# pbs-plus/pbs-plus

Hardware: AMD Instinct MI355X
Metric: GiB/s ingested through CDC+SHA-256 (higher is better)
Workload: dtype u32

## Files before the change

### go/pbsgpu/fallback.go

```go

package pbsgpu

import (
	"errors"
	"io"
	"unsafe"
)

var ErrNotBuilt = errors.New("pbsgpu: built without cgo/gpuchunk; GPU engine unavailable")

var (
	ErrBusy       = errors.New("pbsgpu: all in-flight tickets used")
	ErrHostFaster = errors.New("pbsgpu: too few files in flight for the GPU to beat host SHA-256; hash on the host")
)

const CommIDBytes = 128

type (
	Config struct {
		AvgSize, MinSize, MaxSize, WindowSize int
		BreakTestMask, BreakTestMinimum       uint32
	}
	ChunkInfo struct {
		End     uint64
// ... 22 lines not shown
		Encoded EncodeStats
	}
	ReuseChunk struct {
		Size, Padding, EndOffset uint64
		Digest                   [32]byte
	}
	FileHash    struct{ Index, Size, XXH3 uint64 }
	RingOptions struct {
		ArenaBytes, PageBytes                                                            uint64
		MaxStreams, ShaCUs, RoundPages                                                   uint32
		ExpressCUs                                                                       uint32
		MinRoundPages, MaxInflight, LongBytes, LongLoBytes, LongSpill, PollEvery, Flags uint32
		BacklogMiB, LoneDeferMs, IdleTimeoutS, AutoparkMs                                float64
		LanesCUs                                                                         uint32
		ShortBytes                                                                       uint64
		HoldPages                                                                        bool
	}
	EngineOptions struct {
		Inflight, ShaForm, ShaSlackPct, ShaDensePct                      uint32
		ResolveParMin                                                    uint64
		ShaManyFilesPerCore                                              uint32
		StreamShaCUs, StreamExpressCUs, StreamRingSlots, StreamCtxPool   uint32
		StreamRingGiB                                                    float64
		StreamPageBytes                                                  uint64
	}
	RingStats struct {
		PageBytes, BytesEnqueued, Chunks uint64
		PagesTotal, PagesFree, Rounds    uint32
		ServiceMsLast                    float64
	}
// ... 204 lines not shown
```

### go/pbsgpu/pbsgpu.go

```go

package pbsgpu

import "C"

import (
	"errors"
	"fmt"
	"io"
	"runtime"
	"unsafe"
)

type Config struct {
	AvgSize, MinSize, MaxSize, WindowSize int
	BreakTestMask, BreakTestMinimum       uint32
	c                                     C.pbsgpu_config
}

func NewConfig(avgSize int) (Config, error) {
	var cfg Config
	if st := C.pbsgpu_config_init(C.uint64_t(avgSize), nil, &cfg.c); st != C.PBSGPU_OK {
		return Config{}, fmt.Errorf("buzhash: invalid average chunk size %d: %s", avgSize, strerror(st))
	}
	cfg.AvgSize, cfg.MinSize, cfg.MaxSize = int(cfg.c.avg), int(cfg.c.min), int(cfg.c.max)
// ... 541 lines not shown


type Ring struct {
	h   *C.pbsgpu_ring
	eng *Engine
}

type RingOptions struct {
	ArenaBytes, PageBytes         uint64
	MaxStreams, ShaCUs, RoundPages uint32
	ExpressCUs uint32
	MinRoundPages, MaxInflight, LongBytes, LongLoBytes, LongSpill, PollEvery, Flags uint32
	BacklogMiB, LoneDeferMs, IdleTimeoutS, AutoparkMs                                float64
	LanesCUs   uint32
	ShortBytes uint64
	HoldPages bool
}

const RingOff = ^uint32(0)

func (e *Engine) NewRing(o RingOptions) (*Ring, error) {
	defer runtime.KeepAlive(e)
	co := C.pbsgpu_ring_options{arena_bytes: C.uint64_t(o.ArenaBytes), page_bytes: C.uint64_t(o.PageBytes),
		max_streams: C.uint32_t(o.MaxStreams), sha_cus: C.uint32_t(o.ShaCUs), round_pages: C.uint32_t(o.RoundPages),
		express_cus: C.uint32_t(o.ExpressCUs), min_round_pages: C.uint32_t(o.MinRoundPages),
		max_inflight: C.uint32_t(o.MaxInflight), long_bytes: C.uint32_t(o.LongBytes), long_lo_bytes: C.uint32_t(o.LongLoBytes),
		long_spill: C.uint32_t(o.LongSpill), poll_every: C.uint32_t(o.PollEvery), flags: C.uint32_t(o.Flags),
		backlog_mib: C.double(o.BacklogMiB), lone_defer_ms: C.double(o.LoneDeferMs), idle_timeout_s: C.double(o.IdleTimeoutS),
		autopark_ms: C.double(o.AutoparkMs), lanes_cus: C.uint32_t(o.LanesCUs), short_bytes: C.uint64_t(o.ShortBytes)}
	if o.HoldPages {
		co.flags |= C.PBSGPU_RING_F_HOLD_PAGES
	}
	r := &Ring{eng: e}
	if err := check(C.pbsgpu_ring_create(e.h, &co, &r.h), "ring_create"); err != nil {
		return nil, err
	}
	runtime.SetFinalizer(r, func(r *Ring) { r.Close() })
	return r, nil
}

func (r *Ring) Open() (uint32, error) {
	defer runtime.KeepAlive(r)
	var s C.uint32_t
	st := C.pbsgpu_ring_open(r.h, &s)
// ... 871 lines not shown
```

### include/pbsgpu.h

```cpp
#ifndef PBSGPU_H
#define PBSGPU_H

#include <stddef.h>
#include <stdint.h>

#ifdef __cplusplus
extern "C" {
#endif

#define PBSGPU_ABI_VERSION 5

#define PBSGPU_OK 0
#define PBSGPU_E_INVALID (-1)
#define PBSGPU_E_NO_DEVICE (-2)
#define PBSGPU_E_HIP (-3)
#define PBSGPU_E_NOMEM (-4)
#define PBSGPU_E_CAPACITY (-5)
#define PBSGPU_E_BUSY (-6)
#define PBSGPU_E_TICKET (-7)
#define PBSGPU_E_STATE (-9)

const char *pbsgpu_strerror(int status);
int pbsgpu_abi_version(void);
int pbsgpu_last_hip_error(void);
// ... 128 lines not shown
    uint32_t round_pages;
    uint32_t express_cus;
    uint32_t min_round_pages;
    uint32_t max_inflight;
    uint32_t long_bytes;
    uint32_t long_lo_bytes;
    uint32_t long_spill;
    uint32_t poll_every;
    uint32_t flags;
    uint32_t lanes_cus;
    double backlog_mib;
    double lone_defer_ms;
    double idle_timeout_s;
    double autopark_ms;
    uint64_t short_bytes;
    uint64_t reserved[3];
} pbsgpu_ring_options;
#define PBSGPU_RING_OFF 0xffffffffu
#define PBSGPU_RING_F_NO_OVERLAP 1u
#define PBSGPU_RING_F_NO_STAGE 2u
#define PBSGPU_RING_F_NO_CUT_PRIO 4u
#define PBSGPU_RING_F_NO_SPLIT_AUTO 8u
#define PBSGPU_RING_F_DEFER_SERVICE 16u
#define PBSGPU_RING_F_FILL_SERIAL 32u
#define PBSGPU_RING_F_DENSE_SERVICE 64u
#define PBSGPU_RING_F_DENSE_LANES 128u
#define PBSGPU_RING_F_TIER_TAG 256u
#define PBSGPU_RING_F_HOLD_PAGES 512u
typedef struct pbsgpu_ring_stats {
    uint64_t page_bytes, bytes_enqueued, chunks, candidates, pages_enqueued, pages_recycled, service_bytes_last;
    uint32_t pages_total, pages_free, sha_cus, rounds, rounds_done, rounds_in_flight, streams_opened, service_launches;
// ... 276 lines not shown
```

### pbs_plus_amd/_lib.py

```python
from __future__ import annotations

import ctypes as C
import os
import subprocess

import numpy as np

_HERE = os.path.dirname(os.path.abspath(__file__))
LIB_PATH = os.environ.get("PBSGPU_LIB_PATH") or os.path.join(_HERE, "lib", "libpbsgpu.so")
CSRC = os.path.join(_HERE, "csrc")

OK = 0
E_INVALID, E_NO_DEVICE, E_HIP, E_NOMEM, E_CAPACITY, E_BUSY, E_TICKET, _E_RETIRED_8, E_STATE = range(-1, -10, -1)


class PbsGpuError(RuntimeError):
    def __init__(self, status: int, what: str = ""):
        self.status = status
        msg = lib().pbsgpu_strerror(status).decode() if _lib is not None else str(status)
        hip = lib().pbsgpu_last_hip_error() if _lib is not None else 0
        extra = ""
        if _lib is not None and ("comm" in what or "allgather" in what):
            txt = lib().pbsgpu_comm_last_error()
            if txt:
# ... 53 lines not shown
RING_OFF = 0xFFFFFFFF
RING_F_NO_OVERLAP, RING_F_NO_STAGE, RING_F_NO_CUT_PRIO, RING_F_NO_SPLIT_AUTO, RING_F_DEFER_SERVICE, RING_F_FILL_SERIAL = 1, 2, 4, 8, 16, 32
RING_F_DENSE_SERVICE = 64
RING_F_DENSE_LANES = 128
RING_F_TIER_TAG = 256
RING_F_HOLD_PAGES = 512
RING_ANY_STREAM = 0xFFFFFFFF


class RingOptions(C.Structure):
    _fields_ = [("arena_bytes", C.c_uint64), ("page_bytes", C.c_uint64), ("max_streams", C.c_uint32),
                ("sha_cus", C.c_uint32), ("round_pages", C.c_uint32), ("express_cus", C.c_uint32),
                ("min_round_pages", C.c_uint32), ("max_inflight", C.c_uint32), ("long_bytes", C.c_uint32),
                ("long_lo_bytes", C.c_uint32), ("long_spill", C.c_uint32), ("poll_every", C.c_uint32), ("flags", C.c_uint32),
                ("lanes_cus", C.c_uint32), ("backlog_mib", C.c_double), ("lone_defer_ms", C.c_double),
                ("idle_timeout_s", C.c_double), ("autopark_ms", C.c_double), ("short_bytes", C.c_uint64), ("reserved", C.c_uint64 * 3)]


class EngineOptions(C.Structure):
    _fields_ = [("inflight", C.c_uint32), ("sha_form", C.c_uint32), ("sha_slack_pct", C.c_uint32), ("sha_dense_pct", C.c_uint32),
                ("resolve_par_min", C.c_uint64), ("sha_many_files_per_core", C.c_uint32), ("stream_sha_cus", C.c_uint32),
                ("stream_express_cus", C.c_uint32), ("stream_ring_slots", C.c_uint32), ("stream_ctx_pool", C.c_uint32),
                ("reserved0", C.c_uint32), ("stream_ring_gib", C.c_double), ("stream_page_bytes", C.c_uint64),
                ("reserved", C.c_uint64 * 4)]


class RingStats(C.Structure):
    _fields_ = [(k, C.c_uint64) for k in ("page_bytes", "bytes_enqueued", "chunks", "candidates", "pages_enqueued",
                                          "pages_recycled", "service_bytes_last")] + \
               [(k, C.c_uint32) for k in ("pages_total", "pages_free", "sha_cus", "rounds", "rounds_done",
                                          "rounds_in_flight", "streams_opened", "service_launches")] + \
# ... 222 lines not shown
```

### pbs_plus_amd/csrc/kernels.h

```cpp
#pragma once

#include <hip/hip_runtime.h>
#include <stdint.h>

#include "../../include/pbsgpu.h"

namespace pbsk {

constexpr int kWindow = 64;

struct ScanParams {
    const uint8_t *data_al;
    uint32_t lead;
    uint64_t nbytes;
    uint64_t ntiles;
    uint32_t tile_bytes;
    const uint32_t *table_rot;
    uint32_t thr;
    uint32_t cap;
    uint32_t *tile_cnt;
    uint32_t *tile_slots;
    unsigned long long *tile_queue;
    uint32_t tiles_per_wave;
    uint32_t shared_chip;
// ... 238 lines not shown
    const uint32_t *table_rot;
    const RingPage *pages;
    uint32_t npages;
    const RingSeg *segs_in;
    uint32_t nseg;
    uint32_t seq;
    uint32_t cell_base, cell_cap, cell_mask;
    uint32_t scan_blocks;
    RingRoundStatus *status;
    RingStreamState *streams;
    RingSource q;
    uint4 *desc_w;
    uint4 *ldesc_w;
    uint4 *sdesc_w;
    unsigned long long *tile_queue;
    uint32_t *scalars;
    uint32_t *tile_cnt, *tile_off, *tile_slots, *scan_tmp;
    uint64_t *dense;
    uint64_t dense_cap;
    pbsgpu_segment *segs;
    uint32_t *seg_cnt, *seg_off;
    pbsgpu_record *recs;
    uint64_t rec_cap;
    uint64_t *seg_newc;
    uint32_t *seg_open;
    uint64_t *seg_ecand_in;
    uint64_t *seg_ecand;
    const uint64_t *sugg;
    const uint32_t *sugg_idx;
    uint64_t sugg_feed;
    uint32_t sugg_abs;
    uint32_t pad0;
    const uint32_t *seg_rec_base;
};
struct RingStage {
    const uint8_t *src;
    uint8_t *dst;
    uint32_t off[4], len[4];
    const RingPage *pages_host;
};
hipError_t launch_ring_round(const RingRound &r, int num_cus, hipStream_t st, hipStream_t fill_st = nullptr,
                             hipEvent_t fill_ev = nullptr, hipStream_t scan_st = nullptr, hipEvent_t scan_ev = nullptr,
                             const RingStage *stage = nullptr);
hipError_t launch_ring_service(const RingSource &q, unsigned workgroups, hipStream_t st, bool dense = false);
hipError_t launch_ring_service_xp(const RingSource &q, unsigned workgroups, hipStream_t st);
hipError_t launch_ring_service_lanes(const RingSource &q, unsigned workgroups, hipStream_t st, bool dense);
hipError_t launch_ring_stop(RingCtl *ctl, hipStream_t st);
// ... 13 lines not shown
```

### pbs_plus_amd/csrc/ring.cpp

```cpp
#include <chrono>
#include <cstdio>
#include <cstdlib>
#include <thread>

#include "ring_internal.h"

using namespace pbse;

namespace {

double now_ms() {
    return std::chrono::duration<double, std::milli>(std::chrono::steady_clock::now().time_since_epoch()).count();
}

uint32_t pow2_at_least(uint64_t v) {
    uint32_t p = 1;
    while (p < v && p < (1u << 31)) p <<= 1;
    return p;
}

volatile uint32_t *hb_words(const pbsgpu_ring *r) { return r->heartbeat.as<volatile uint32_t>(); }

void ring_service_ended(pbsgpu_ring *r) {
    if (r->svc == SvcState::Stopped) return;
// ... 184 lines not shown
        if (inflight > 0 && !any_final && ready < r->min_round_pages) return PBSGPU_OK;
        if (inflight >= r->max_inflight) return PBSGPU_OK;
    }
    int in = -1;
    for (uint32_t i = 0; i < kRingInputs; ++i)
        if (!r->input_busy[i]) { in = (int)i; break; }
    if (in < 0) return PBSGPU_OK;
    {
        const uint64_t oldest = r->rounds.empty() ? r->cell_cursor : r->rounds.front().cell_base;
        if (r->cell_cursor + r->rec_cap - oldest > r->ncells) return PBSGPU_OK;
    }
    pbsk::RingPage *pg = r->in_pages((uint32_t)in);
    pbsk::RingSeg *sg = r->in_segs((uint32_t)in);
    uint32_t *recbase = r->in_recbase((uint32_t)in);
    uint32_t *suggidx = r->in_suggidx((uint32_t)in);
    uint32_t np = 0, ns = 0;
    uint64_t cells_needed = 0, new_bytes = 0;
    RoundInfo ri;
    std::vector<hipEvent_t> deps;
    std::vector<uint64_t> sugg;
    const uint32_t minsz = std::min(e->effmin, e->cfg.min);
    const uint64_t feed = e->sugg_feed.load(std::memory_order_relaxed);
    const uint64_t look = feed > 1 ? (uint64_t)e->cfg.max : 0;
    uint32_t streams_waiting = 0;
    for (auto &s : r->slots) streams_waiting += (s.open && !s.ready.empty()) ? 1u : 0u;
    const uint32_t round_cap = (r->svc == SvcState::Stopped || streams_waiting < 2)
                                   ? r->round_pages
                                   : std::max(std::min(r->round_pages, r->min_round_pages), r->round_pages / 2);
    for (uint32_t si = 0; si < r->slots.size() && np < round_cap; ++si) {
        StreamSlot &s = r->slots[si];
        if (!s.open || (s.ready.empty() && !s.zero_final)) continue;
// ... 3 lines not shown
        g.reset = s.fresh ? 1u : 0u;
        g.origin = s.origin;
        const uint64_t end_old = s.bytes_enqueued;
        uint64_t end = end_old;
        uint32_t take = 0;
        while (!s.ready.empty() && take < kPagesPerStreamRound && np < round_cap) {
            const PageReq &q = s.ready.front();
            pbsk::RingPage p{};
            p.phys = q.phys;
            p.phys_off = (uint64_t)q.phys * r->stride + 128u;
            p.logical = ((uint64_t)si << pbsk::kRingOffBits) | (q.k * r->page_bytes);
            p.valid = q.valid;
            p.slot = si;
            p.seg = ns;
            p.do_fill = q.do_fill ? 1u : 0u;
            p.fill_seed = q.seed;
            p.fill_off = q.fill_off;
            p.fill_kind = q.kind;
            p.fill_tab = q.tab;
            p.fill_ntab = q.ntab;
            p.prev_phys = (q.k > 0 && s.last_phys >= 0) ? (uint32_t)s.last_phys : 0xffffffffu;
            s.last_phys = (int64_t)q.phys;
            pg[np++] = p;
            if (q.dep) deps.push_back(q.dep);
            end += q.valid;
            new_bytes += q.valid;
            if (q.final) g.final = 1;
            s.ready.pop_front();
            ++take;
        }
// ... 75 lines not shown
    rr.nseg = ns;
    rr.seq = ri.seq;
    rr.cell_base = (uint32_t)(ri.cell_base & (r->ncells - 1));
    rr.cell_cap = ri.cell_cap;
    rr.cell_mask = r->ncells - 1;
    rr.scan_blocks = (uint32_t)std::max(1, e->num_cus - (int)r->svc_cus);
    rr.status = hs;
    rr.streams = r->streams.as<pbsk::RingStreamState>();
    rr.q = r->source();
    rr.desc_w = r->desc.as<uint4>();
    rr.ldesc_w = r->ldesc.as<uint4>();
    rr.sdesc_w = r->lanes_cus ? r->sdesc.as<uint4>() : nullptr;
    const uint32_t set = r->ps ? r->scan_set : 0u;
    rr.scalars = r->scalars.as<uint32_t>();
    rr.tile_queue = r->tileq.as<unsigned long long>() + set * 8u;
    rr.tile_cnt = set ? r->tile_cnt2.as<uint32_t>() : r->tile_cnt.as<uint32_t>();
    rr.tile_off = r->tile_off.as<uint32_t>();
    rr.tile_slots = set ? r->tile_slots2.as<uint32_t>() : r->tile_slots.as<uint32_t>();
    rr.scan_tmp = r->scan_tmp.as<uint32_t>();
    rr.dense = r->dense.as<uint64_t>();
    rr.dense_cap = r->dense_cap;
    rr.segs = r->segs.as<pbsgpu_segment>();
    rr.seg_cnt = r->seg_cnt.as<uint32_t>();
    rr.seg_off = r->seg_off.as<uint32_t>();
    rr.recs = r->recs.as<pbsgpu_record>();
    rr.rec_cap = r->rec_cap;
    rr.seg_newc = r->seg_newc.as<uint64_t>();
    rr.seg_open = r->seg_open.as<uint32_t>();
    rr.seg_ecand_in = r->seg_ecand_in.as<uint64_t>();
    rr.seg_ecand = r->seg_ecand.as<uint64_t>();
// ... 5 lines not shown
    std::atomic_thread_fence(std::memory_order_release);
    bool defer = r->defer_service;
    if (!defer && r->svc == SvcState::Stopped && r->lone_defer_ms > 0 && !any_final &&
        np >= std::max<uint32_t>(1, r->round_pages / 2)) {
        const uint64_t lanes_worth = (uint64_t)r->sha_cus * (r->dense_service ? 256u : 128u) * (uint64_t)e->cfg.avg;
        const double t = now_ms();
        if (r->defer_t0 == 0) r->defer_t0 = t;
        defer = t - r->defer_t0 < r->lone_defer_ms && r->deferred_bytes + new_bytes < lanes_worth;
    }
    if (!defer) {
        const int st = ring_start_service(r);
        if (st != PBSGPU_OK) return fail(st);
        rr.q = r->source();
    }
    if (r->svc == SvcState::Stopped) r->deferred_bytes += new_bytes;
    if (r->svc == SvcState::Stopped) rr.scan_blocks = (uint32_t)std::max(1, e->num_cus);
    else if (r->ps && rr.scan_blocks > 8) rr.scan_blocks -= 1;
    hipStream_t scan_st = r->ps ? r->ps : r->cs;
    for (hipEvent_t ev : deps)
        if (hipStreamWaitEvent(scan_st, ev, 0) != hipSuccess) return fail(PBSGPU_E_HIP);
    for (hipEvent_t ev : deps) ring_event_put(r, ev);
    deps.clear();
    if (r->ps && r->ctl_used[set])
        if (hipStreamWaitEvent(r->ps, r->ev_ctl[set], 0) != hipSuccess) return fail(PBSGPU_E_HIP);
    {
        const bool fill_serial = r->fill_serial;
        pbsk::RingStage stg{};
        if (r->stage_inputs) {
            const uint8_t *hb = r->in((uint32_t)in);
            uint8_t *db = r->in_dev((uint32_t)in);
            stg.src = hb;
            stg.dst = db;
            stg.off[0] = (uint32_t)r->in_pages_off;   stg.len[0] = np * (uint32_t)sizeof(pbsk::RingPage);
            stg.off[1] = (uint32_t)r->in_segs_off;    stg.len[1] = ns * (uint32_t)sizeof(pbsk::RingSeg);
            stg.off[2] = (uint32_t)r->in_recbase_off; stg.len[2] = (ns + 1u) * 4u;
            stg.off[3] = (uint32_t)r->in_suggidx_off; stg.len[3] = rr.sugg_idx ? (ns + 1u) * 4u : 0u;
            stg.pages_host = pg;
            auto mirror = [&](const void *hp) { return db + (reinterpret_cast<const uint8_t *>(hp) - hb); };
            rr.pages = reinterpret_cast<const pbsk::RingPage *>(mirror(pg));
            rr.segs_in = reinterpret_cast<const pbsk::RingSeg *>(mirror(sg));
            rr.seg_rec_base = reinterpret_cast<const uint32_t *>(mirror(recbase));
// ... 41 lines not shown
    enum Kind { U32, U32_ZERO_OFF, U64, F64, F64_ZERO_NEG, FLAG_IF_ZERO, FLAG_IF_SET };
    struct Entry {
        const char *name;
        Kind kind;
        void *field;
        uint32_t flag;
    };
    const Entry table[] = {
        {"PBSGPU_RING_SHA_CUS", U32, &o.sha_cus, 0},
        {"PBSGPU_RING_XP_CUS", U32_ZERO_OFF, &o.express_cus, 0},
        {"PBSGPU_RING_LANES_CUS", U32, &o.lanes_cus, 0},
        {"PBSGPU_RING_SHORT_BYTES", U64, &o.short_bytes, 0},
        {"PBSGPU_RING_ROUND_PAGES", U32, &o.round_pages, 0},
        {"PBSGPU_RING_MIN_ROUND_PAGES", U32, &o.min_round_pages, 0},
        {"PBSGPU_RING_MAX_INFLIGHT", U32, &o.max_inflight, 0},
        {"PBSGPU_RING_LONG_BYTES", U32_ZERO_OFF, &o.long_bytes, 0},
        {"PBSGPU_RING_LONG_LO_BYTES", U32_ZERO_OFF, &o.long_lo_bytes, 0},
        {"PBSGPU_RING_LONG_SPILL", U32, &o.long_spill, 0},
        {"PBSGPU_RING_POLL_EVERY", U32, &o.poll_every, 0},
        {"PBSGPU_RING_BACKLOG_MIB", F64_ZERO_NEG, &o.backlog_mib, 0},
        {"PBSGPU_RING_LONE_DEFER_MS", F64_ZERO_NEG, &o.lone_defer_ms, 0},
        {"PBSGPU_RING_IDLE_TIMEOUT_S", F64, &o.idle_timeout_s, 0},
        {"PBSGPU_RING_AUTOPARK_MS", F64, &o.autopark_ms, 0},
        {"PBSGPU_RING_OVERLAP", FLAG_IF_ZERO, &o.flags, PBSGPU_RING_F_NO_OVERLAP},
        {"PBSGPU_RING_STAGE_INPUTS", FLAG_IF_ZERO, &o.flags, PBSGPU_RING_F_NO_STAGE},
        {"PBSGPU_RING_CUT_PRIO", FLAG_IF_ZERO, &o.flags, PBSGPU_RING_F_NO_CUT_PRIO},
        {"PBSGPU_RING_SPLIT_AUTO", FLAG_IF_ZERO, &o.flags, PBSGPU_RING_F_NO_SPLIT_AUTO},
        {"PBSGPU_RING_DEFER_SERVICE", FLAG_IF_SET, &o.flags, PBSGPU_RING_F_DEFER_SERVICE},
        {"PBSGPU_RING_FILL_SERIAL", FLAG_IF_SET, &o.flags, PBSGPU_RING_F_FILL_SERIAL},
        {"PBSGPU_RING_DENSE_SERVICE", FLAG_IF_SET, &o.flags, PBSGPU_RING_F_DENSE_SERVICE},
// ... 204 lines not shown
                                               : std::max(1u, r->round_pages / 4);
        r->backlog_limit = o.backlog_mib < 0 ? 0 : o.backlog_mib > 0 ? (uint64_t)(o.backlog_mib * 1048576.0)   : (uint64_t)(r->sha_cus + r->lanes_cus) << 27;
        r->backlog_auto = o.backlog_mib == 0;
        if (o.max_inflight) r->max_inflight = std::min<uint32_t>(std::max(1u, o.max_inflight), kRingInputs);
        r->autopark_ms = std::max(0.0, o.autopark_ms);
        r->defer_service = (o.flags & PBSGPU_RING_F_DEFER_SERVICE) != 0;
        r->fill_serial = (o.flags & PBSGPU_RING_F_FILL_SERIAL) != 0;
        r->dense_service = (o.flags & PBSGPU_RING_F_DENSE_SERVICE) != 0;
        r->dense_lanes = (o.flags & PBSGPU_RING_F_DENSE_LANES) != 0;
        r->tier_tag = (o.flags & PBSGPU_RING_F_TIER_TAG) != 0;
        r->lone_defer_ms = o.lone_defer_ms < 0 ? 0.0 : o.lone_defer_ms > 0 ? o.lone_defer_ms : 25.0;
        r->idle_timeout_s = o.idle_timeout_s;
        r->opt_long_lo = o.long_lo_bytes;
        r->opt_long_spill = o.long_spill;
        r->opt_poll_every = o.poll_every;
        const double lambda = 3.0 * r->tile_bytes / ((double)e->cfg.mask + 1.0);
        uint32_t capv = 8;
        while (capv < 4.0 * lambda + 16.0) capv <<= 1;
        r->cap = std::min<uint32_t>(std::max<uint32_t>(capv * 2, r->tile_bytes / 128), r->tile_bytes);
        const uint64_t ntiles = (uint64_t)r->round_pages * r->tpp;
        if (ntiles * r->cap >= (1ull << 32)) return PBSGPU_E_INVALID;
        const uint32_t minsz = std::min(e->effmin, e->cfg.min);
        r->dense_cap = ntiles * r->cap;
        r->rec_cap = ((uint64_t)r->round_pages * r->page_bytes + (uint64_t)r->max_streams * e->cfg.max) / minsz +
                     4ull * r->max_streams + 64;
        const uint64_t resident_chunks = (uint64_t)r->npages * r->page_bytes / minsz + 2ull * r->npages + r->rec_cap;
        r->qslots = pow2_at_least(2 * resident_chunks + 4096);
        r->ncells = pow2_at_least(4 * resident_chunks + 4 * r->rec_cap);
        r->nfree = pow2_at_least(4ull * r->npages + 64);

// ... 3 lines not shown
        CHK(r->streams.ensure((size_t)r->max_streams * sizeof(pbsk::RingStreamState)));
        CHK(r->pending.ensure((size_t)r->npages * 4 + 64));
        CHK(r->desc.ensure((size_t)r->qslots * 32));
        r->long_bytes = r->xp_cus ? (long_bytes_hint ? long_bytes_hint : (uint32_t)((uint64_t)e->cfg.max * 13 / 16)) : 0;
        r->long_lo_auto = long_bytes_hint == 0;
        if (o.long_bytes) r->long_bytes = o.long_bytes == PBSGPU_RING_OFF ? 0u : o.long_bytes;
        if (r->xp_cus && r->long_bytes == 0) r->xp_cus = 0;
        r->lslots = pow2_at_least(2 * ((uint64_t)r->npages * r->page_bytes / std::max<uint32_t>(r->long_bytes, minsz) + r->rec_cap) + 1024);
        CHK(r->ldesc.ensure((size_t)r->lslots * 32));
        r->sslots = r->lanes_cus ? r->qslots : 2;
        CHK(r->sdesc.ensure((size_t)r->sslots * 32));
        CHK(r->scalars.ensure(pbsk::kRsCount * 4 + 64));
        CHK(r->tile_cnt.ensure((size_t)ntiles * 4 + 16));
        CHK(r->tile_off.ensure((size_t)ntiles * 4 + 16));
        CHK(r->tile_slots.ensure((size_t)ntiles * r->cap * 4 + 16));
        CHK(r->tileq.ensure(128));
        const bool overlap = !(o.flags & PBSGPU_RING_F_NO_OVERLAP);
        if (overlap) {
            CHK(r->tile_cnt2.ensure((size_t)ntiles * 4 + 16));
            CHK(r->tile_slots2.ensure((size_t)ntiles * r->cap * 4 + 16));
        }
        CHK(r->dense.ensure((size_t)r->dense_cap * 8 + 16));
        CHK(r->scan_tmp.ensure(pbsk::scan_tmp_words(std::max<uint64_t>(ntiles, r->max_streams)) * 4 + 64));
        CHK(r->segs.ensure((size_t)r->max_streams * sizeof(pbsgpu_segment)));
        CHK(r->seg_cnt.ensure((size_t)r->max_streams * 4 + 16));
        CHK(r->seg_off.ensure((size_t)r->max_streams * 4 + 16));
        CHK(r->seg_newc.ensure((size_t)r->max_streams * 8 + 16));
        CHK(r->seg_open.ensure((size_t)r->max_streams * 4 + 16));
        CHK(r->seg_ecand_in.ensure((size_t)r->max_streams * 8 + 16));
        CHK(r->seg_ecand.ensure((size_t)r->max_streams * 8 + 16));
        CHK(r->recs.ensure((size_t)r->rec_cap * sizeof(pbsgpu_record) + 64));
// ... 12 lines not shown
        CHK(r->inputs.ensure(r->input_stride * kRingInputs));
        r->stage_inputs = !(o.flags & PBSGPU_RING_F_NO_STAGE);
        if (r->stage_inputs) CHK(r->inputs_dev.ensure(r->input_stride * kRingInputs));
        std::memset(r->inputs.p, 0, r->input_stride * kRingInputs);
        int prio_lo = 0, prio_hi = 0;
        HIPCHK(hipDeviceGetStreamPriorityRange(&prio_lo, &prio_hi));
        const bool cut_prio = !(o.flags & PBSGPU_RING_F_NO_CUT_PRIO);
        r->bulk_prio = cut_prio ? prio_lo : 0;
        HIPCHK(hipStreamCreateWithFlags(&r->cs, hipStreamNonBlocking));
        HIPCHK(hipStreamCreateWithPriority(&r->fs, hipStreamNonBlocking, r->bulk_prio));
        HIPCHK(hipMemsetAsync(r->ctl.p, 0, 256, r->cs));
        HIPCHK(hipMemsetAsync(r->probe.p, 0, 128, r->cs));
        HIPCHK(hipMemsetAsync(r->streams.p, 0, (size_t)r->max_streams * sizeof(pbsk::RingStreamState), r->cs));
        HIPCHK(hipMemsetAsync(r->pending.p, 0, (size_t)r->npages * 4 + 64, r->cs));
        HIPCHK(hipMemsetAsync(r->scalars.p, 0, pbsk::kRsCount * 4 + 64, r->cs));
        HIPCHK(hipMemsetAsync(r->tileq.p, 0, 128, r->cs));
        HIPCHK(hipStreamSynchronize(r->cs));
        for (auto &ev : r->ev_fill) HIPCHK(hipEventCreateWithFlags(&ev, hipEventDisableTiming));
        if (overlap) {
            HIPCHK(hipStreamCreateWithPriority(&r->ps, hipStreamNonBlocking, r->bulk_prio));
            for (auto &ev : r->ev_scan) HIPCHK(hipEventCreateWithFlags(&ev, hipEventDisableTiming));
            for (auto &ev : r->ev_ctl) HIPCHK(hipEventCreateWithFlags(&ev, hipEventDisableTiming));
        }
        int lo = 0, hi = 0;
        HIPCHK(hipDeviceGetStreamPriorityRange(&lo, &hi));
        HIPCHK(hipStreamCreateWithPriority(&r->ss, hipStreamNonBlocking, hi));
        if (r->xp_cus) {
            HIPCHK(hipStreamCreateWithPriority(&r->xs, hipStreamNonBlocking, hi));
            HIPCHK(hipEventCreateWithFlags(&r->ev_xsvc1, hipEventDisableTiming));
        }
        if (r->lanes_cus) {
// ... 617 lines not shown
```

### pbs_plus_amd/csrc/ring_internal.h

```cpp
#pragma once

#include <deque>
#include <mutex>
#include <vector>

#include "engine_internal.h"
#include "hold.h"

namespace pbse {

constexpr uint32_t kRingInputs = 16;
constexpr uint32_t kPagesPerStreamRound = 256;

struct PageReq {
    uint32_t phys = 0;
    uint64_t k = 0;
    uint32_t valid = 0;
    bool final = false;
    bool do_fill = false;
    uint64_t seed = 0, fill_off = 0;
    uint32_t kind = 0;
    const pbsk::FillPiece *tab = nullptr;
    uint32_t ntab = 0;
    hipEvent_t dep = nullptr;
// ... 90 lines not shown
    uint32_t rounds_enq = 0;
    double autopark_ms = 0;
    double idle_since_ms = 0;
    bool dense_service = false;
    bool dense_lanes = false;
    bool tier_tag = false;
    bool backlog_auto = true;
    uint32_t park_gen_seen = 0;
    uint32_t park_grace_gen = 0;
    double park_wait_t0 = 0;
    bool parked_for_flush = false;
    bool fill_serial = false;
    bool hold = false;
    pbse::HeldPages held;
    uint32_t opt_long_lo = 0, opt_long_spill = 0, opt_poll_every = 0;
    bool defer_service = false;
    double lone_defer_ms = 25.0;
    double defer_t0 = 0;
    uint64_t deferred_bytes = 0;
    double idle_timeout_s = 0;
    std::vector<uint32_t> free_pages;
    uint32_t free_read = 0;
    std::vector<pbse::StreamSlot> slots;
    std::deque<pbse::RoundInfo> rounds;
    bool input_busy[pbse::kRingInputs] = {};
    uint32_t next_seq = 1;
    uint64_t cell_cursor = 0;
    int error = PBSGPU_OK;
    pbsgpu_ring_stats st{};
    double svc_t0 = 0;
// ... 55 lines not shown
```

### pbs_plus_amd/csrc/ring_kernels.inc

```

__device__ __forceinline__ bool ring_short_ticket(const RingRound &r, const RingDesc &d) {
    const uint32_t idx = atomicAdd(&r.scalars[kRsNshort], 1u);
    if (idx >= r.scalars[kRsShortRoom]) return false;
    ring_desc_encode(r.sdesc_w, (r.q.ctl->stail + idx) & r.q.smask, d);
    return true;
}

__global__ __launch_bounds__(256) void k_ring_fill(RingRound r) {
    const RingPage &pe = r.pages[blockIdx.y];
    if (!pe.do_fill) return;
    uint64_t *dst = reinterpret_cast<uint64_t *>(r.arena + pe.phys_off);
    const uint64_t nwords = ((uint64_t)pe.valid + 7u) / 8u;
    const uint64_t w0 = pe.fill_off >> 3;
    const uint64_t stride = (uint64_t)gridDim.x * blockDim.x;
    if (pe.fill_kind == 4u) {
        uint4 *d4 = reinterpret_cast<uint4 *>(dst);
        const uint32_t nblk = (uint32_t)((nwords + 1u) / 2u), step = gridDim.x * blockDim.x;
        const uint64_t q0 = w0 >> 1;
        uint32_t i = blockIdx.x * blockDim.x + threadIdx.x;
        for (; i + 3u * step < nblk; i += 4u * step) {
            const uint4 a = chacha2_block(q0 + i, pe.fill_seed), b = chacha2_block(q0 + i + step, pe.fill_seed);
            const uint4 c = chacha2_block(q0 + i + 2u * step, pe.fill_seed), d = chacha2_block(q0 + i + 3u * step, pe.fill_seed);
            d4[i] = a;
            d4[i + step] = b;
            d4[i + 2u * step] = c;
            d4[i + 3u * step] = d;
        }
        for (; i < nblk; i += step) d4[i] = chacha2_block(q0 + i, pe.fill_seed);
        return;
    }
    if (pe.fill_kind == 5u) {
        uint4 *d4 = reinterpret_cast<uint4 *>(dst);
        const uint32_t nblk = (uint32_t)((nwords + 1u) / 2u), step = gridDim.x * blockDim.x;
        const FillPiece *tab = pe.fill_tab;
        const uint32_t nt = pe.fill_ntab;
        FillPiece pc{~0ull, 0, 0, 0};
        for (uint32_t i = blockIdx.x * blockDim.x + threadIdx.x; i < nblk; i += step) {
            const uint64_t x = pe.fill_off + 16ull * i;
            if (!(x >= pc.dst_off && x - pc.dst_off < pc.len)) {
                uint32_t lo = 0, hi = nt;
                while (hi - lo > 1u) {
                    const uint32_t mid = (lo + hi) >> 1;
                    if (tab[mid].dst_off <= x) lo = mid; else hi = mid;
                }
                pc = tab[lo];
            }
            d4[i] = chacha2_block((pc.src_off + (x - pc.dst_off)) >> 4, pc.seed);
        }
        return;
    }
    for (uint64_t i = (uint64_t)blockIdx.x * blockDim.x + threadIdx.x; i < nwords; i += stride)
        dst[i] = fill_word(w0 + i, pe.fill_seed, pe.fill_kind);
}

__global__ __launch_bounds__(64) void k_ring_prep_pages(RingRound r) {
    const uint32_t b = blockIdx.x;
    const int t = threadIdx.x;
    if (b == 0 && t == 0) *r.tile_queue = 0ull;
    if (b >= r.npages || t >= 8) return;
    const RingPage &pe = r.pages[b];
    uint4 v = make_uint4(0, 0, 0, 0);
    if (pe.prev_phys != 0xffffffffu)
        v = reinterpret_cast<const uint4 *>(r.arena + (uint64_t)pe.prev_phys * r.stride + 128u + r.page_bytes - 128)[t];
    reinterpret_cast<uint4 *>(r.arena + pe.phys_off - 128)[t] = v;
}

__global__ __launch_bounds__(64) void k_ring_prep(RingRound r) {
    const uint32_t b = blockIdx.x;
    const int t = threadIdx.x;
    if (b == 0 && t < kRsCount) {
        uint32_t v = 0;
        if (t == kRsShortRoom && r.q.short_bytes) {
            const unsigned long long sq = __hip_atomic_load(&r.q.ctl->sq, __ATOMIC_RELAXED, __HIP_MEMORY_SCOPE_AGENT);
            const uint32_t waiting = (uint32_t)sq - (uint32_t)(sq >> 32);
            v = waiting < r.q.short_room ? r.q.short_room - waiting : 0u;
        }
        r.scalars[t] = v;
    }
    if (b < r.npages) {
        const RingPage &pe = r.pages[b];
        const RingSeg &sg = r.segs_in[pe.seg];
        RingStreamState *st = r.streams + pe.slot;
        const uint64_t off = pe.logical & kRingOffMask;
        const uint64_t k = off / r.page_bytes;
        const uint8_t *body = r.arena + pe.phys_off;
        const uint8_t *prev = nullptr;
        if (b > sg.first_page) {
            prev = r.arena + r.pages[b - 1].phys_off;
        } else if (k > 0 && !sg.reset && st->c < off) {
            prev = r.arena + (uint64_t)st->pt[(k - 1) % kRingPT] * r.stride + 128u;
        }
        if (t < 8 && prev) {
            uint4 *tailpad = reinterpret_cast<uint4 *>(const_cast<uint8_t *>(prev) + r.page_bytes);
            tailpad[t] = reinterpret_cast<const uint4 *>(body)[t];
        }
        if (t == 32) st->pt[k % kRingPT] = pe.phys;
        return;
    }
    const uint32_t s = b - r.npages;
    if (s >= r.nseg || t != 0) return;
    const RingSeg &sg = r.segs_in[s];
    const RingStreamState *st = r.streams + sg.slot;
    const uint64_t c = sg.reset ? 0ull : st->c;
    r.segs[s].offset = ((uint64_t)sg.slot << kRingOffBits) | c;
    r.segs[s].length = sg.new_end - c;
    r.seg_newc[s] = c;
    r.seg_open[s] = (sg.new_end > c && !sg.final) ? 1u : 0u;
    r.seg_ecand_in[s] = sg.reset ? ~0ull : st->ecand;
    r.seg_ecand[s] = ~0ull;
}

__device__ __forceinline__ void ring_order_one(const RingRound &r, const uint32_t i, const pbsgpu_record &rec, const uint32_t s,
                                               const bool is_last) {
    const RingSeg &sg = r.segs_in[s];
    const RingStreamState *st = r.streams + sg.slot;
    const uint64_t Aoff = r.segs[s].offset & kRingOffMask;
    const uint64_t endl = Aoff + rec.end, start = endl - rec.size;
    const uint32_t cell = (r.cell_base + i) & r.cell_mask;
    uint32_t *cw = reinterpret_cast<uint32_t *>(r.q.cells + (uint64_t)cell * kCellBytes);
    if (is_last && r.seg_open[s]) {
        cw[kCellSize] = 0;
        return;
    }
    const uint64_t G = r.page_bytes;
// ... 134 lines not shown
    }
    for (uint32_t j = 0; j < c; ++j) {
        const uint32_t vj = sl[j];
        const uint32_t pos = cnt[min((vj - 1u) / strip, 63u)]++;
        if (base + pos < r.dense_cap) r.dense[base + pos] = tbase + vj;
    }
}

__global__ __launch_bounds__(1024) void k_ring_control(RingRound r, SuggFeed fr) {
    __shared__ uint32_t wsum[16];
    __shared__ uint32_t err_s, n_s;
    const uint32_t tid = threadIdx.x;
    const int lane = tid & 63, wave = tid >> 6;
    RingCtl *ctl = r.q.ctl;
    const unsigned long long tk0 = wall_clock64();
    const uint64_t ntiles = (uint64_t)r.npages * r.tpp;
    const uint64_t per = (ntiles + 1023u) / 1024u;
    const uint64_t t0 = min((uint64_t)tid * per, ntiles), t1 = min(t0 + per, ntiles);
    uint32_t mine = 0, over = 0;
    for (uint64_t tb = t0; tb < t1; tb += 16u) {
        uint32_t v[16];
#pragma unroll
        for (int j = 0; j < 16; ++j) v[j] = (tb + j < t1) ? r.tile_cnt[tb + j] : 0u;
#pragma unroll
        for (int j = 0; j < 16; ++j) {
            over |= (v[j] > r.cap) ? 1u : 0u;
            mine += min(v[j], r.cap);
        }
    }
    uint32_t ncand = 0;
// ... 134 lines not shown
    for (uint32_t i = blockIdx.x * blockDim.x + threadIdx.x; i < n16; i += gridDim.x * blockDim.x) b[i] = a[i];
}

hipError_t launch_ring_round(const RingRound &r, int num_cus, hipStream_t st, hipStream_t fill_st, hipEvent_t fill_ev,
                             hipStream_t scan_st, hipEvent_t scan_ev, const RingStage *stage) {
    hipStream_t sst = scan_st ? scan_st : st;
    bool any_fill = false;
    const RingPage *hp = stage ? stage->pages_host : r.pages;
    for (uint32_t i = 0; i < r.npages; ++i) any_fill |= hp[i].do_fill != 0;
    if (stage) {
        uint32_t mx = 1;
        for (int k = 0; k < 4; ++k) mx = std::max(mx, (stage->len[k] / 16u + 255u) / 256u);
        hipLaunchKernelGGL(k_ring_stage, dim3(std::min(mx, 8u), 4), dim3(256), kRingLdsTag, (any_fill && fill_st) ? fill_st : sst, *stage);
    }
    if (any_fill) {
        hipLaunchKernelGGL(k_ring_fill, dim3(16, r.npages), dim3(256), kRingLdsTag, fill_st ? fill_st : sst, r);
        if (fill_st && fill_st != sst) {
            hipError_t e = hipEventRecord(fill_ev, fill_st);
            if (e != hipSuccess) return e;
            e = hipStreamWaitEvent(sst, fill_ev, 0);
            if (e != hipSuccess) return e;
        }
    }
    hipLaunchKernelGGL(k_ring_prep_pages, dim3(r.npages ? r.npages : 1), dim3(64), kRingLdsTag, sst, r);
    const uint64_t ntiles = (uint64_t)r.npages * r.tpp;
    if (ntiles) {
        ScanParams p{};
        p.data_al = r.arena;
        p.lead = 0;
        p.nbytes = ~0ull >> 1;
        p.ntiles = ntiles;
// ... 4 lines not shown
        p.tile_cnt = r.tile_cnt;
        p.tile_slots = r.tile_slots;
        p.tile_queue = r.tile_queue;
        p.ring_pages = r.pages;
        p.ring_tpp = r.tpp;
        p.max_blocks = r.scan_blocks;
        hipError_t e = (r.tile_bytes == 64u * 34u * 128u) ? launch_scan3_any<34>(p, num_cus, sst) : launch_scan3_any<4>(p, num_cus, sst);
        if (e != hipSuccess) return e;
    }
    if (sst != st) {
        hipError_t e = hipEventRecord(scan_ev, sst);
        if (e != hipSuccess) return e;
        e = hipStreamWaitEvent(st, scan_ev, 0);
        if (e != hipSuccess) return e;
    }
    hipLaunchKernelGGL(k_ring_prep, dim3(r.npages + r.nseg), dim3(64), kRingLdsTag, st, r);
    hipLaunchKernelGGL(k_ring_control, dim3(1), dim3(1024), kRingLdsTag, st, r, SuggFeed{r.sugg_feed, 0, r.sugg_abs, 0});
    return hipGetLastError();
}

hipError_t launch_ring_service_xp(const RingSource &q, unsigned workgroups, hipStream_t st) {
    hipFuncAttributes fa{};
    hipError_t e = hipFuncGetAttributes(&fa, reinterpret_cast<const void *>(&k_sha256_xpair<RingSource>));
    if (e != hipSuccess) return e;
    size_t pad = (160u << 10) > fa.sharedSizeBytes ? (160u << 10) - fa.sharedSizeBytes : 0;
    pad &= ~(size_t)255;
    e = allow_lds(&k_sha256_xpair<RingSource>, pad);
    if (e != hipSuccess) return e;
    hipLaunchKernelGGL((k_sha256_xpair<RingSource>), dim3(workgroups), dim3(256), pad, st, q, (const uint32_t *)nullptr, 0u,
                       (uint32_t *)nullptr, (const uint32_t *)nullptr);
    return hipGetLastError();
// ... 27 lines not shown
```

Before: 651.0.

## Persistent work-queue ring fill kernel with CU partitioning and prep folded into control

```diff
diff --git a/go/pbsgpu/fallback.go b/go/pbsgpu/fallback.go
--- a/go/pbsgpu/fallback.go
+++ b/go/pbsgpu/fallback.go
@@ -60,6 +60,7 @@
 		BacklogMiB, LoneDeferMs, IdleTimeoutS, AutoparkMs                                float64
 		LanesCUs                                                                         uint32
 		ShortBytes                                                                       uint64
+		FillCUs                                                                          uint32
 		HoldPages                                                                        bool
 	}
 	EngineOptions struct {
diff --git a/go/pbsgpu/pbsgpu.go b/go/pbsgpu/pbsgpu.go
--- a/go/pbsgpu/pbsgpu.go
+++ b/go/pbsgpu/pbsgpu.go
@@ -579,6 +579,7 @@
 	BacklogMiB, LoneDeferMs, IdleTimeoutS, AutoparkMs                                float64
 	LanesCUs   uint32
 	ShortBytes uint64
+	FillCUs uint32
 	HoldPages bool
 }
 
@@ -592,7 +593,8 @@
 		max_inflight: C.uint32_t(o.MaxInflight), long_bytes: C.uint32_t(o.LongBytes), long_lo_bytes: C.uint32_t(o.LongLoBytes),
 		long_spill: C.uint32_t(o.LongSpill), poll_every: C.uint32_t(o.PollEvery), flags: C.uint32_t(o.Flags),
 		backlog_mib: C.double(o.BacklogMiB), lone_defer_ms: C.double(o.LoneDeferMs), idle_timeout_s: C.double(o.IdleTimeoutS),
-		autopark_ms: C.double(o.AutoparkMs), lanes_cus: C.uint32_t(o.LanesCUs), short_bytes: C.uint64_t(o.ShortBytes)}
+		autopark_ms: C.double(o.AutoparkMs), lanes_cus: C.uint32_t(o.LanesCUs), short_bytes: C.uint64_t(o.ShortBytes),
+		fill_cus: C.uint32_t(o.FillCUs)}
 	if o.HoldPages {
 		co.flags |= C.PBSGPU_RING_F_HOLD_PAGES
 	}
diff --git a/include/pbsgpu.h b/include/pbsgpu.h
--- a/include/pbsgpu.h
+++ b/include/pbsgpu.h
@@ -166,7 +166,9 @@
     double idle_timeout_s;
     double autopark_ms;
     uint64_t short_bytes;
-    uint64_t reserved[3];
+    uint32_t fill_cus;
+    uint32_t reserved1;
+    uint64_t reserved[2];
 } pbsgpu_ring_options;
 #define PBSGPU_RING_OFF 0xffffffffu
 #define PBSGPU_RING_F_NO_OVERLAP 1u
diff --git a/pbs_plus_amd/_lib.py b/pbs_plus_amd/_lib.py
--- a/pbs_plus_amd/_lib.py
+++ b/pbs_plus_amd/_lib.py
@@ -91,7 +91,8 @@
                 ("min_round_pages", C.c_uint32), ("max_inflight", C.c_uint32), ("long_bytes", C.c_uint32),
                 ("long_lo_bytes", C.c_uint32), ("long_spill", C.c_uint32), ("poll_every", C.c_uint32), ("flags", C.c_uint32),
                 ("lanes_cus", C.c_uint32), ("backlog_mib", C.c_double), ("lone_defer_ms", C.c_double),
-                ("idle_timeout_s", C.c_double), ("autopark_ms", C.c_double), ("short_bytes", C.c_uint64), ("reserved", C.c_uint64 * 3)]
+                ("idle_timeout_s", C.c_double), ("autopark_ms", C.c_double), ("short_bytes", C.c_uint64), ("fill_cus", C.c_uint32),
+                ("reserved1", C.c_uint32), ("reserved", C.c_uint64 * 2)]
 
 
 class EngineOptions(C.Structure):
diff --git a/pbs_plus_amd/csrc/kernels.h b/pbs_plus_amd/csrc/kernels.h
--- a/pbs_plus_amd/csrc/kernels.h
+++ b/pbs_plus_amd/csrc/kernels.h
@@ -276,6 +276,7 @@
     uint4 *ldesc_w;
     uint4 *sdesc_w;
     unsigned long long *tile_queue;
+    unsigned long long *fill_queue;
     uint32_t *scalars;
     uint32_t *tile_cnt, *tile_off, *tile_slots, *scan_tmp;
     uint64_t *dense;
@@ -292,7 +293,9 @@
     const uint32_t *sugg_idx;
     uint64_t sugg_feed;
     uint32_t sugg_abs;
-    uint32_t pad0;
+    uint32_t fill_blocks;
+    uint32_t fill_shared;
+    uint32_t pad1;
     const uint32_t *seg_rec_base;
 };
 struct RingStage {
diff --git a/pbs_plus_amd/csrc/ring.cpp b/pbs_plus_amd/csrc/ring.cpp
--- a/pbs_plus_amd/csrc/ring.cpp
+++ b/pbs_plus_amd/csrc/ring.cpp
@@ -222,7 +222,7 @@
     pbsk::RingSeg *sg = r->in_segs((uint32_t)in);
     uint32_t *recbase = r->in_recbase((uint32_t)in);
     uint32_t *suggidx = r->in_suggidx((uint32_t)in);
-    uint32_t np = 0, ns = 0;
+    uint32_t np = 0, ns = 0, fill_pages = 0;
     uint64_t cells_needed = 0, new_bytes = 0;
     RoundInfo ri;
     std::vector<hipEvent_t> deps;
@@ -256,6 +256,7 @@
             p.slot = si;
             p.seg = ns;
             p.do_fill = q.do_fill ? 1u : 0u;
+            fill_pages += p.do_fill;
             p.fill_seed = q.seed;
             p.fill_off = q.fill_off;
             p.fill_kind = q.kind;
@@ -361,6 +362,7 @@
     const uint32_t set = r->ps ? r->scan_set : 0u;
     rr.scalars = r->scalars.as<uint32_t>();
     rr.tile_queue = r->tileq.as<unsigned long long>() + set * 8u;
+    rr.fill_queue = r->tileq.as<unsigned long long>() + 16u + (uint32_t)in;
     rr.tile_cnt = set ? r->tile_cnt2.as<uint32_t>() : r->tile_cnt.as<uint32_t>();
     rr.tile_off = r->tile_off.as<uint32_t>();
     rr.tile_slots = set ? r->tile_slots2.as<uint32_t>() : r->tile_slots.as<uint32_t>();
@@ -396,8 +398,28 @@
         rr.q = r->source();
     }
     if (r->svc == SvcState::Stopped) r->deferred_bytes += new_bytes;
-    if (r->svc == SvcState::Stopped) rr.scan_blocks = (uint32_t)std::max(1, e->num_cus);
-    else if (r->ps && rr.scan_blocks > 8) rr.scan_blocks -= 1;
+    if (fill_pages) r->rounds_since_fill = 0;
+    else if (r->rounds_since_fill < 1000u) r->rounds_since_fill++;
+    bool fill_serial = r->fill_serial;
+    if (r->svc == SvcState::Stopped) {
+        rr.scan_blocks = (uint32_t)std::max(1, e->num_cus);
+        rr.fill_blocks = 2u * rr.scan_blocks;
+        rr.fill_shared = 1;
+    } else {
+        constexpr uint32_t kFillRecent = 8;
+        const int cut = std::max(1, e->num_cus - (int)r->svc_cus);
+        const int rest = cut - ((r->ps && cut > 8) ? 1 : 0);
+        if (r->opt_fill_cus && !fill_serial && rest >= 2) {
+            const int F = r->rounds_since_fill < kFillRecent ? (int)std::min<uint32_t>(r->opt_fill_cus, (uint32_t)rest - 1u) : 0;
+            rr.scan_blocks = (uint32_t)(rest - F);
+            rr.fill_blocks = (uint32_t)std::max(1, F);
+        } else {
+            fill_serial = true;
+            rr.scan_blocks = (uint32_t)std::max(1, rest);
+            rr.fill_blocks = 2u * rr.scan_blocks;
+            rr.fill_shared = 1;
+        }
+    }
     hipStream_t scan_st = r->ps ? r->ps : r->cs;
     for (hipEvent_t ev : deps)
         if (hipStreamWaitEvent(scan_st, ev, 0) != hipSuccess) return fail(PBSGPU_E_HIP);
@@ -406,7 +428,6 @@
     if (r->ps && r->ctl_used[set])
         if (hipStreamWaitEvent(r->ps, r->ev_ctl[set], 0) != hipSuccess) return fail(PBSGPU_E_HIP);
     {
-        const bool fill_serial = r->fill_serial;
         pbsk::RingStage stg{};
         if (r->stage_inputs) {
             const uint8_t *hb = r->in((uint32_t)in);
@@ -478,6 +499,7 @@
         {"PBSGPU_RING_ROUND_PAGES", U32, &o.round_pages, 0},
         {"PBSGPU_RING_MIN_ROUND_PAGES", U32, &o.min_round_pages, 0},
         {"PBSGPU_RING_MAX_INFLIGHT", U32, &o.max_inflight, 0},
+        {"PBSGPU_RING_FILL_CUS", U32, &o.fill_cus, 0},
         {"PBSGPU_RING_LONG_BYTES", U32_ZERO_OFF, &o.long_bytes, 0},
         {"PBSGPU_RING_LONG_LO_BYTES", U32_ZERO_OFF, &o.long_lo_bytes, 0},
         {"PBSGPU_RING_LONG_SPILL", U32, &o.long_spill, 0},
@@ -712,6 +734,7 @@
         r->opt_long_lo = o.long_lo_bytes;
         r->opt_long_spill = o.long_spill;
         r->opt_poll_every = o.poll_every;
+        r->opt_fill_cus = o.fill_cus;
         const double lambda = 3.0 * r->tile_bytes / ((double)e->cfg.mask + 1.0);
         uint32_t capv = 8;
         while (capv < 4.0 * lambda + 16.0) capv <<= 1;
@@ -745,7 +768,7 @@
         CHK(r->tile_cnt.ensure((size_t)ntiles * 4 + 16));
         CHK(r->tile_off.ensure((size_t)ntiles * 4 + 16));
         CHK(r->tile_slots.ensure((size_t)ntiles * r->cap * 4 + 16));
-        CHK(r->tileq.ensure(128));
+        CHK(r->tileq.ensure(128 + kRingInputs * 8));
         const bool overlap = !(o.flags & PBSGPU_RING_F_NO_OVERLAP);
         if (overlap) {
             CHK(r->tile_cnt2.ensure((size_t)ntiles * 4 + 16));
@@ -788,7 +811,7 @@
         HIPCHK(hipMemsetAsync(r->streams.p, 0, (size_t)r->max_streams * sizeof(pbsk::RingStreamState), r->cs));
         HIPCHK(hipMemsetAsync(r->pending.p, 0, (size_t)r->npages * 4 + 64, r->cs));
         HIPCHK(hipMemsetAsync(r->scalars.p, 0, pbsk::kRsCount * 4 + 64, r->cs));
-        HIPCHK(hipMemsetAsync(r->tileq.p, 0, 128, r->cs));
+        HIPCHK(hipMemsetAsync(r->tileq.p, 0, 128 + kRingInputs * 8, r->cs));
         HIPCHK(hipStreamSynchronize(r->cs));
         for (auto &ev : r->ev_fill) HIPCHK(hipEventCreateWithFlags(&ev, hipEventDisableTiming));
         if (overlap) {
diff --git a/pbs_plus_amd/csrc/ring_internal.h b/pbs_plus_amd/csrc/ring_internal.h
--- a/pbs_plus_amd/csrc/ring_internal.h
+++ b/pbs_plus_amd/csrc/ring_internal.h
@@ -128,6 +128,8 @@
     bool hold = false;
     pbse::HeldPages held;
     uint32_t opt_long_lo = 0, opt_long_spill = 0, opt_poll_every = 0;
+    uint32_t opt_fill_cus = 0;
+    uint32_t rounds_since_fill = 1000;
     bool defer_service = false;
     double lone_defer_ms = 25.0;
     double defer_t0 = 0;
diff --git a/pbs_plus_amd/csrc/ring_kernels.inc b/pbs_plus_amd/csrc/ring_kernels.inc
--- a/pbs_plus_amd/csrc/ring_kernels.inc
+++ b/pbs_plus_amd/csrc/ring_kernels.inc
@@ -6,57 +6,76 @@
     return true;
 }
 
-__global__ __launch_bounds__(256) void k_ring_fill(RingRound r) {
-    const RingPage &pe = r.pages[blockIdx.y];
-    if (!pe.do_fill) return;
-    uint64_t *dst = reinterpret_cast<uint64_t *>(r.arena + pe.phys_off);
-    const uint64_t nwords = ((uint64_t)pe.valid + 7u) / 8u;
-    const uint64_t w0 = pe.fill_off >> 3;
-    const uint64_t stride = (uint64_t)gridDim.x * blockDim.x;
-    if (pe.fill_kind == 4u) {
-        uint4 *d4 = reinterpret_cast<uint4 *>(dst);
-        const uint32_t nblk = (uint32_t)((nwords + 1u) / 2u), step = gridDim.x * blockDim.x;
-        const uint64_t q0 = w0 >> 1;
-        uint32_t i = blockIdx.x * blockDim.x + threadIdx.x;
-        for (; i + 3u * step < nblk; i += 4u * step) {
-            const uint4 a = chacha2_block(q0 + i, pe.fill_seed), b = chacha2_block(q0 + i + step, pe.fill_seed);
-            const uint4 c = chacha2_block(q0 + i + 2u * step, pe.fill_seed), d = chacha2_block(q0 + i + 3u * step, pe.fill_seed);
-            d4[i] = a;
-            d4[i + step] = b;
-            d4[i + 2u * step] = c;
-            d4[i + 3u * step] = d;
-        }
-        for (; i < nblk; i += step) d4[i] = chacha2_block(q0 + i, pe.fill_seed);
-        return;
-    }
-    if (pe.fill_kind == 5u) {
-        uint4 *d4 = reinterpret_cast<uint4 *>(dst);
-        const uint32_t nblk = (uint32_t)((nwords + 1u) / 2u), step = gridDim.x * blockDim.x;
-        const FillPiece *tab = pe.fill_tab;
-        const uint32_t nt = pe.fill_ntab;
-        FillPiece pc{~0ull, 0, 0, 0};
-        for (uint32_t i = blockIdx.x * blockDim.x + threadIdx.x; i < nblk; i += step) {
-            const uint64_t x = pe.fill_off + 16ull * i;
-            if (!(x >= pc.dst_off && x - pc.dst_off < pc.len)) {
-                uint32_t lo = 0, hi = nt;
-                while (hi - lo > 1u) {
-                    const uint32_t mid = (lo + hi) >> 1;
-                    if (tab[mid].dst_off <= x) lo = mid; else hi = mid;
+constexpr unsigned kRingFillLds = 96u << 10;
+constexpr uint32_t kRingFillSlice = 128u << 10;
+__global__ __launch_bounds__(1024) void k_ring_fill(RingRound r) {
+    __shared__ unsigned long long ticket[2];
+    const uint32_t tid = threadIdx.x;
+    const uint32_t spp = (r.page_bytes + kRingFillSlice - 1u) / kRingFillSlice;
+    const unsigned long long nitems = (unsigned long long)r.npages * spp;
+    unsigned long long next = 0;
+    if (tid == 0) ticket[0] = atomicAdd(r.fill_queue, 1ull);
+    __syncthreads();
+    for (uint32_t it = 0;; ++it) {
+        const unsigned long long item = ticket[it & 1u];
+        if (item >= nitems) break;
+        if (tid == 0) next = atomicAdd(r.fill_queue, 1ull);
+        const RingPage &pe = r.pages[item / spp];
+        const uint32_t sl = (uint32_t)(item % spp);
+        if (pe.do_fill) {
+            uint64_t *dst = reinterpret_cast<uint64_t *>(r.arena + pe.phys_off);
+            const uint64_t nwords = ((uint64_t)pe.valid + 7u) / 8u;
+            const uint64_t w0 = pe.fill_off >> 3;
+            const uint32_t nblk = (uint32_t)((nwords + 1u) / 2u);
+            const uint32_t b0 = sl * (kRingFillSlice / 16u), b1 = min(nblk, b0 + kRingFillSlice / 16u);
+            if (pe.fill_kind == 4u) {
+                uint4 *d4 = reinterpret_cast<uint4 *>(dst);
+                constexpr uint32_t step = 1024u;
+                const uint64_t q0 = w0 >> 1;
+                uint32_t i = b0 + tid;
+                for (; i + 3u * step < b1; i += 4u * step) {
+                    const uint4 a = chacha2_block(q0 + i, pe.fill_seed), b = chacha2_block(q0 + i + step, pe.fill_seed);
+                    const uint4 c = chacha2_block(q0 + i + 2u * step, pe.fill_seed), d = chacha2_block(q0 + i + 3u * step, pe.fill_seed);
+                    d4[i] = a;
+                    d4[i + step] = b;
+                    d4[i + 2u * step] = c;
+                    d4[i + 3u * step] = d;
                 }
-                pc = tab[lo];
+                for (; i < b1; i += step) d4[i] = chacha2_block(q0 + i, pe.fill_seed);
+            } else if (pe.fill_kind == 5u) {
+                uint4 *d4 = reinterpret_cast<uint4 *>(dst);
+                const FillPiece *tab = pe.fill_tab;
+                const uint32_t nt = pe.fill_ntab;
+                FillPiece pc{~0ull, 0, 0, 0};
+                for (uint32_t i = b0 + tid; i < b1; i += 1024u) {
+                    const uint64_t x = pe.fill_off + 16ull * i;
+                    if (!(x >= pc.dst_off && x - pc.dst_off < pc.len)) {
+                        uint32_t lo = 0, hi = nt;
+                        while (hi - lo > 1u) {
+                            const uint32_t mid = (lo + hi) >> 1;
+                            if (tab[mid].dst_off <= x) lo = mid; else hi = mid;
+                        }
+                        pc = tab[lo];
+                    }
+                    d4[i] = chacha2_block((pc.src_off + (x - pc.dst_off)) >> 4, pc.seed);
+                }
+            } else {
+                const uint64_t e = min(nwords, 2ull * b1);
+                for (uint64_t i = 2ull * b0 + tid; i < e; i += 1024u) dst[i] = fill_word(w0 + i, pe.fill_seed, pe.fill_kind);
             }
-            d4[i] = chacha2_block((pc.src_off + (x - pc.dst_off)) >> 4, pc.seed);
-        }
-        return;
-    }
-    for (uint64_t i = (uint64_t)blockIdx.x * blockDim.x + threadIdx.x; i < nwords; i += stride)
-        dst[i] = fill_word(w0 + i, pe.fill_seed, pe.fill_kind);
+        }
+        if (tid == 0) ticket[(it + 1u) & 1u] = next;
+        __syncthreads();
+    }
 }
 
 __global__ __launch_bounds__(64) void k_ring_prep_pages(RingRound r) {
     const uint32_t b = blockIdx.x;
     const int t = threadIdx.x;
-    if (b == 0 && t == 0) *r.tile_queue = 0ull;
+    if (b == 0 && t == 0) {
+        *r.tile_queue = 0ull;
+        *r.fill_queue = 0ull;
+    }
     if (b >= r.npages || t >= 8) return;
     const RingPage &pe = r.pages[b];
     uint4 v = make_uint4(0, 0, 0, 0);
@@ -65,19 +84,18 @@
     reinterpret_cast<uint4 *>(r.arena + pe.phys_off - 128)[t] = v;
 }
 
-__global__ __launch_bounds__(64) void k_ring_prep(RingRound r) {
-    const uint32_t b = blockIdx.x;
-    const int t = threadIdx.x;
-    if (b == 0 && t < kRsCount) {
+__device__ __forceinline__ void ring_prep(const RingRound &r, const uint32_t tid) {
+    if (tid < (uint32_t)kRsCount) {
         uint32_t v = 0;
-        if (t == kRsShortRoom && r.q.short_bytes) {
+        if (tid == (uint32_t)kRsShortRoom && r.q.short_bytes) {
             const unsigned long long sq = __hip_atomic_load(&r.q.ctl->sq, __ATOMIC_RELAXED, __HIP_MEMORY_SCOPE_AGENT);
             const uint32_t waiting = (uint32_t)sq - (uint32_t)(sq >> 32);
             v = waiting < r.q.short_room ? r.q.short_room - waiting : 0u;
         }
-        r.scalars[t] = v;
-    }
-    if (b < r.npages) {
+        r.scalars[tid] = v;
+    }
+    const uint32_t t = tid & 15u;
+    for (uint32_t b = tid >> 4; b < r.npages; b += 64u) {
         const RingPage &pe = r.pages[b];
         const RingSeg &sg = r.segs_in[pe.seg];
         RingStreamState *st = r.streams + pe.slot;
@@ -94,20 +112,19 @@
             uint4 *tailpad = reinterpret_cast<uint4 *>(const_cast<uint8_t *>(prev) + r.page_bytes);
             tailpad[t] = reinterpret_cast<const uint4 *>(body)[t];
         }
-        if (t == 32) st->pt[k % kRingPT] = pe.phys;
-        return;
-    }
-    const uint32_t s = b - r.npages;
-    if (s >= r.nseg || t != 0) return;
-    const RingSeg &sg = r.segs_in[s];
-    const RingStreamState *st = r.streams + sg.slot;
-    const uint64_t c = sg.reset ? 0ull : st->c;
-    r.segs[s].offset = ((uint64_t)sg.slot << kRingOffBits) | c;
-    r.segs[s].length = sg.new_end - c;
-    r.seg_newc[s] = c;
-    r.seg_open[s] = (sg.new_end > c && !sg.final) ? 1u : 0u;
-    r.seg_ecand_in[s] = sg.reset ? ~0ull : st->ecand;
-    r.seg_ecand[s] = ~0ull;
+        if (t == 8) st->pt[k % kRingPT] = pe.phys;
+    }
+    for (uint32_t s = tid; s < r.nseg; s += 1024u) {
+        const RingSeg &sg = r.segs_in[s];
+        const RingStreamState *st = r.streams + sg.slot;
+        const uint64_t c = sg.reset ? 0ull : st->c;
+        r.segs[s].offset = ((uint64_t)sg.slot << kRingOffBits) | c;
+        r.segs[s].length = sg.new_end - c;
+        r.seg_newc[s] = c;
+        r.seg_open[s] = (sg.new_end > c && !sg.final) ? 1u : 0u;
+        r.seg_ecand_in[s] = sg.reset ? ~0ull : st->ecand;
+        r.seg_ecand[s] = ~0ull;
+    }
 }
 
 __device__ __forceinline__ void ring_order_one(const RingRound &r, const uint32_t i, const pbsgpu_record &rec, const uint32_t s,
@@ -272,6 +289,9 @@
     const int lane = tid & 63, wave = tid >> 6;
     RingCtl *ctl = r.q.ctl;
     const unsigned long long tk0 = wall_clock64();
+    ring_prep(r, tid);
+    __threadfence();
+    __syncthreads();
     const uint64_t ntiles = (uint64_t)r.npages * r.tpp;
     const uint64_t per = (ntiles + 1023u) / 1024u;
     const uint64_t t0 = min((uint64_t)tid * per, ntiles), t1 = min(t0 + per, ntiles);
@@ -436,7 +456,10 @@
         hipLaunchKernelGGL(k_ring_stage, dim3(std::min(mx, 8u), 4), dim3(256), kRingLdsTag, (any_fill && fill_st) ? fill_st : sst, *stage);
     }
     if (any_fill) {
-        hipLaunchKernelGGL(k_ring_fill, dim3(16, r.npages), dim3(256), kRingLdsTag, fill_st ? fill_st : sst, r);
+        hipError_t fe = allow_lds(&k_ring_fill, kRingFillLds);
+        if (fe != hipSuccess) return fe;
+        hipLaunchKernelGGL(k_ring_fill, dim3(std::max(1u, r.fill_blocks)), dim3(1024), r.fill_shared ? kRingLdsTag : kRingFillLds,
+                           fill_st ? fill_st : sst, r);
         if (fill_st && fill_st != sst) {
             hipError_t e = hipEventRecord(fill_ev, fill_st);
             if (e != hipSuccess) return e;
@@ -471,7 +494,6 @@
         e = hipStreamWaitEvent(st, scan_ev, 0);
         if (e != hipSuccess) return e;
     }
-    hipLaunchKernelGGL(k_ring_prep, dim3(r.npages + r.nseg), dim3(64), kRingLdsTag, st, r);
     hipLaunchKernelGGL(k_ring_control, dim3(1), dim3(1024), kRingLdsTag, st, r, SuggFeed{r.sugg_feed, 0, r.sugg_abs, 0});
     return hipGetLastError();
 }
```

Result: faster. 710.1, median of 6 (+9.1%).
